# FedericoCos/PathTracer_GaussianSplatting

Hardware: AMD Instinct MI355X
Metric: Mrays/s (path trace) + Gsplats/s (3DGS) at 1920×1080, 1/2/4/8 MI355X (higher is better)
Workload: dtype f32; 1 GPU; C3 path trace: 250000-tri Sponza-like atrium, 1920x1080, 64 spp per GPU; width=1920, height=1080, spp_per_gpu=64, triangles=250000, bvh_nodes=58627, bvh_depth=13, bvh_build=host binned SAH, 103.2 ms, parallelism=single GPU

## Files before the change

### pathtracer_gaussiansplatting_amd/csrc/api.cpp

```cpp
#ifndef PTGS_BVH_LEAF
#define PTGS_BVH_LEAF 3
#endif
#include <hip/hip_runtime.h>

#include <algorithm>
#include <chrono>
#include <cmath>
#include <cstdarg>
#include <cstdio>
#include <cstring>
#include <string>
#include <vector>

#include "../../include/ptgs/ptgs.h"
#include "bvh.h"
#include "bvh_gpu.h"
#include "knn.h"
#include "hostmath.h"
#include "pt_launch.h"
#include "pt_wavefront.h"
#include "comm.h"
#include "splat.h"
#include "splat_backward.h"
#include "splat_sh.h"
// ... 396 lines not shown
      (void)hipFree(g.tri_flags);
    } else {
      (void)hipFree(g.nodes);
      (void)hipFree(g.tris);
      (void)hipFree(g.tri_flags);
      return fail(c, PTGS_EHIP, "GPU BVH build: %s", hipGetErrorString(e));
    }
  }
  if (!built) {
    auto t0 = std::chrono::steady_clock::now();
    BvhOut bvh;
    std::vector<float> n4;
    uint32_t num4 = 0, dep4 = 0, need = PTGS_STACK_TOTAL;
    int built_leaf = -1;
    bool fits = false;
    uint32_t built_depth = 0;
    for (const BvhTry& tr : bvh_tries()) {
      if (tr.leaf != built_leaf || tr.depth != built_depth) {
        build_bvh(tris, tr.leaf, tr.depth, bvh);
        built_leaf = tr.leaf;
        built_depth = tr.depth;
        if (bvh.depth >= PTGS_STACK) return fail(c, PTGS_ERANGE, "BVH depth %u exceeds the traversal stack", bvh.depth);
      }
      fits = collapse_fit(bvh.nodes, n4, num4, dep4, tr.fan, need);
      bvh_log("host", tr.leaf, tr.fan, tr.depth, dep4, need);
      if (fits) break;
    }
    auto t1 = std::chrono::steady_clock::now();
    if (!fits) return fail(c, PTGS_ERANGE, "BVH depth %u exceeds the traversal stack", bvh.depth);
    s.deep_stack = need >= PTGS_STACK ? 1 : 0;
    if ((rc = upload(c, (const float4*)n4.data(), n4.size() / 4, &s.nodes))) return rc;
    host_n4.swap(n4);
    bvh.num_nodes = num4;
    bvh.depth = dep4;
    if ((rc = upload(c, (const float4*)bvh.tris.data(), bvh.tris.size() / 4, &s.tris))) return rc;
    if ((rc = upload(c, bvh.tri_flags.data(), bvh.tri_flags.size(), &s.tri_flags))) return rc;
    c->info.num_bvh_nodes = bvh.num_nodes;
    c->info.bvh_depth = bvh.depth;
    c->info.max_leaf_size = bvh.max_leaf;
    c->info.build_ms = std::chrono::duration<double, std::milli>(t1 - t0).count();
  }
  if (c->info.num_bvh_nodes > bvh_node_limit())
    return fail(c, PTGS_ERANGE, "BVH of %u 4-wide nodes exceeds the traversal's 2 GiB node window (%u nodes)",
                c->info.num_bvh_nodes, bvh_node_limit());
  {
    const size_t nf = (size_t)c->info.num_bvh_nodes * 32;
    if (host_n4.size() != nf) {
      host_n4.resize(nf);
      HIPCHK(c, hipMemcpy(host_n4.data(), s.nodes, nf * sizeof(float), hipMemcpyDeviceToHost));
    }
    std::vector<uint32_t> n64;
    if (!quantize_bvh4(host_n4.data(), c->info.num_bvh_nodes, n64))
      return fail(c, PTGS_ERANGE, "BVH node extents beyond the compact nodes' step range (2^-100 .. 2^100)");
    if ((rc = upload(c, (const uint4*)n64.data(), n64.size() / 4, &s.nodes64))) return rc;
  }
  ptgs_vertex dummy_v{};
  uint32_t dummy_i = 0;
  ptgs_mesh_info dummy_m{};
  if ((rc = upload(c, d->num_vertices ? d->vertices : &dummy_v, d->num_vertices ? d->num_vertices : 1, &s.vertices))) return rc;
  if ((rc = upload(c, d->num_indices ? d->indices : &dummy_i, d->num_indices ? d->num_indices : 1, &s.indices))) return rc;
  if ((rc = upload(c, d->num_meshes ? d->meshes : &dummy_m, d->num_meshes ? d->num_meshes : 1, &s.meshes))) return rc;
  if ((rc = upload(c, d->materials, d->num_materials, &s.materials))) return rc;
  {
    const uint32_t zero4[4] = {0, 0, 0, 0};
    if ((rc = upload(c, (const uint4*)(hitrec.empty() ? zero4 : hitrec.data()), hitrec.empty() ? 1 : hitrec.size() / 4,
                     &s.hitrec)))
      return rc;
  }
  if ((rc = upload(c, d->light_triangles, d->num_light_triangles, &s.light_tris))) return rc;
  if ((rc = upload(c, d->light_cdf, d->num_light_cdf, &s.light_cdf))) return rc;
  if ((rc = upload(c, d->punctual_lights, d->num_punctual_lights, &s.plights))) return rc;
  if ((rc = upload(c, d->punctual_cdf, d->num_punctual_cdf, &s.pcdf))) return rc;
  if ((rc = upload(c, (const float4*)d->blue_noise_rgba32f, (size_t)bn * bn, &s.blue_noise))) return rc;
  if ((rc = upload(c, texpool.texels.data(), texpool.texels.size(), &s.tex.texels))) return rc;
  if ((rc = upload(c, texpool.info.data(), texpool.info.size(), &s.tex.info))) return rc;
  if ((rc = upload(c, texpool.lut.data(), texpool.lut.size(), &s.tex.lut))) return rc;
  s.tex.count = d->num_textures;
  s.uses_textures = 0;
  for (uint32_t i = 0; i < d->num_materials; ++i) {
    const ptgs_material& m = d->materials[i];
    if (m.albedo_texture_index > 0 || m.normal_texture_index > 0 || m.metallic_roughness_texture_index > 0 ||
        m.emissive_texture_index > 0 || m.clearcoat_texture_index > 0 || m.clearcoat_roughness_texture_index > 0 ||
        m.sg_id > 0)
      s.uses_textures = 1;
  }
  s.num_light_cdf = d->num_light_cdf;
  s.num_plights = d->num_punctual_lights;
  s.bn_size = (int32_t)bn;
  s.has_transparent = has_transparent ? 1 : 0;
  c->dsc = s;
  c->has_scene = true;
  c->info.num_triangles = (uint32_t)tris.size();
  return PTGS_OK;
}

int ptgs_scene_get_info(const ptgs_ctx* c, ptgs_scene_info* out) {
  if (!c || !out) return PTGS_EINVAL;
  if (!c->has_scene) return PTGS_ENOSCENE;
  *out = c->info;
  return PTGS_OK;
}

int ptgs_scene_get_bvh(const ptgs_ctx* c, ptgs_bvh_buffers* out) {
  if (!c || !out) return PTGS_EINVAL;
  if (!c->has_scene) return PTGS_ENOSCENE;
  out->nodes = (const float*)c->dsc.nodes;
// ... 585 lines not shown
```

### pathtracer_gaussiansplatting_amd/csrc/bvh.cpp

```cpp
#include "bvh.h"

#include <algorithm>
#include <cmath>
#include <cstring>
#include <limits>

#ifndef PTGS_BVH_CT
#define PTGS_BVH_CT 0.125f
#endif
#ifndef PTGS_BVH_BINS
#define PTGS_BVH_BINS 32
#endif

namespace ptgs {

namespace {

struct Box {
  float lo[3], hi[3];
  void reset() {
    for (int a = 0; a < 3; ++a) { lo[a] = std::numeric_limits<float>::infinity(); hi[a] = -lo[a]; }
  }
  void grow(const float* p) {
    for (int a = 0; a < 3; ++a) { lo[a] = std::min(lo[a], p[a]); hi[a] = std::max(hi[a], p[a]); }
// ... 289 lines not shown
    const float* f = &n4[32 * (size_t)i];
    uint32_t* o = &out[PTGS_NODE64_DWORDS * (size_t)i];
    bool real[4];
    for (int j = 0; j < 4; ++j) {
      real[j] = true;
      for (int a = 0; a < 3; ++a) {
        const float lo = f[(2 * a) * 4 + j], hi = f[(2 * a + 1) * 4 + j];
        if (!(std::fabs(lo) < kFar && std::fabs(hi) < kFar && lo <= hi)) real[j] = false;
      }
    }
    for (int a = 0; a < 3; ++a) {
      const float* lo = f + (2 * a) * 4;
      const float* hi = f + (2 * a + 1) * 4;
      float lmin = std::numeric_limits<float>::infinity(), hmax = -lmin;
      for (int j = 0; j < 4; ++j)
        if (real[j]) { lmin = std::min(lmin, lo[j]); hmax = std::max(hmax, hi[j]); }
      float org = 0.0f, step = 1.0f;
      uint32_t wlo = 0xffffffffu, whi = 0u;
      if (lmin <= hmax) {
        org = std::nextafterf((float)((double)lmin - m), -std::numeric_limits<float>::infinity());
        int e = (int)std::ceil(std::log2(std::max(((double)hmax + m - (double)org) / 255.0, 1e-300)));
        e = std::max(e, -100);
        for (;; ++e) {
          if (e > 100) return false;
          step = std::ldexp(1.0f, e);
          bool fits = true;
          wlo = 0xffffffffu; whi = 0u;
          for (int j = 0; j < 4 && fits; ++j) {
            if (!real[j]) continue;
            const double tl = (double)lo[j] - m, th = (double)hi[j] + m;
            double ql = std::floor((tl - (double)org) / (double)step);
            ql = std::min(std::max(ql, 0.0), 255.0);
            while (ql > 0.0 && (double)std::fmaf((float)ql, step, org) > tl) ql -= 1.0;
            double qh = std::ceil((th - (double)org) / (double)step);
            qh = std::min(std::max(qh, 0.0), 256.0);
            while (qh <= 255.0 && (double)std::fmaf((float)qh, step, org) < th) qh += 1.0;
            if (qh > 255.0) { fits = false; break; }
            wlo = (wlo & ~(0xffu << (8 * j))) | ((uint32_t)ql << (8 * j));
            whi |= (uint32_t)qh << (8 * j);
          }
          if (fits) break;
        }
      }
      std::memcpy(&o[a], &org, 4);
      std::memcpy(&o[3 + a], &step, 4);
      o[6 + 2 * a] = wlo;
      o[7 + 2 * a] = whi;
    }
    std::memcpy(&o[12], &f[24], 16);
  }
  return true;
}

}
```

### pathtracer_gaussiansplatting_amd/csrc/bvh.h

```cpp
#pragma once

#include <stdint.h>
#include <vector>

namespace ptgs {

struct BuildTri {
  float v0[3], v1[3], v2[3];
  uint32_t mesh, prim, gid;
  uint32_t flags;
};

struct BvhOut {
  std::vector<float> nodes;
  std::vector<float> tris;
  std::vector<uint32_t> tri_flags;
  uint32_t num_nodes = 0;
  uint32_t depth = 0;
  uint32_t max_leaf = 0;
};

void build_bvh(const std::vector<BuildTri>& tris, int max_leaf_size, uint32_t max_depth, BvhOut& out);

void collapse_bvh4(const std::vector<float>& nodes2, std::vector<float>& nodes4, uint32_t& num_nodes4,
                   uint32_t& max_stack, uint32_t& depth4, int max_children = 4);

#define PTGS_NODE64_DWORDS 16
bool quantize_bvh4(const float* nodes4, uint32_t num_nodes, std::vector<uint32_t>& out);

}
```

### pathtracer_gaussiansplatting_amd/csrc/pt_device.h

```cpp
#pragma once

#include <hip/hip_runtime.h>
#include "detmath.h"
#include "texture.h"
#include "../../include/ptgs/ptgs.h"

namespace ptgs {

struct DevScene {
  const float4* nodes;
  const uint4* nodes64;
  const float4* tris;
  const uint32_t* tri_flags;
  const ptgs_vertex* vertices;
  const uint32_t* indices;
  const ptgs_mesh_info* meshes;
  const ptgs_material* materials;
  const uint4* hitrec;
  const ptgs_light_triangle* light_tris;
  const ptgs_light_cdf* light_cdf;
  const ptgs_punctual_light* plights;
  const ptgs_punctual_cdf* pcdf;
  const float4* blue_noise;
  DevTextures tex;
  int32_t uses_textures;
  int32_t deep_stack;
  uint32_t num_light_cdf;
  uint32_t num_plights;
  int32_t bn_size;
  int32_t has_transparent;
};

struct CamParams {
  float inv_view[16];
  float inv_proj[16];
  float ambient[4];
  float emissive_flux, punctual_flux, p_emissive;
  float fov, win_height, use_lod, lod_factor;
};

struct Hit {
  float t, u, v;
  uint32_t gid;
  uint32_t slot;
};

struct TraversalCounters {
  uint32_t nodes;
  uint32_t tris;
  uint32_t hits;
#ifdef PT_LANES
  struct PtLaneCounts* lanes_p;
#endif
};

enum PtLoop { PT_L_NODE = 0, PT_L_LEAF, PT_L_TRI, PT_L_ANY_NODE, PT_L_ANY_TRI, PT_L_BOUNCE, PT_L_SAMPLE, PT_L_COUNT };
#ifdef PT_LANES
__device__ unsigned long long g_pt_lanes[2 * PT_L_COUNT];
struct PtLaneCounts {
  uint32_t w[PT_L_COUNT], l[PT_L_COUNT];
};
__device__ __forceinline__ void pt_lane_tick(PtLaneCounts& c, int i) {
  const unsigned long long ex = __builtin_amdgcn_read_exec();
  c.l[i] += 1u;
  if (__lane_id() == (uint32_t)__builtin_ctzll(ex)) c.w[i] += 1u;
}
__device__ __forceinline__ void pt_lanes_flush(const PtLaneCounts& c) {
  for (int i = 0; i < PT_L_COUNT; ++i) {
    atomicAdd(&g_pt_lanes[2 * i], (unsigned long long)c.w[i]);
    atomicAdd(&g_pt_lanes[2 * i + 1], (unsigned long long)c.l[i]);
  }
}
#define PT_LANE_TICK(cnt, i) pt_lane_tick(*(cnt).lanes_p, (i))
#define PT_LANES_INIT(tc) PtLaneCounts tc##_lanes = {}; (tc).lanes_p = &tc##_lanes
#define PT_LANES_FLUSH(tc) pt_lanes_flush(tc##_lanes)
#else
#define PT_LANE_TICK(cnt, i) ((void)0)
#define PT_LANES_INIT(tc) ((void)0)
#define PT_LANES_FLUSH(tc) ((void)0)
#endif

#ifndef PTGS_STACK
#define PTGS_STACK 39
// ... 51 lines not shown
#if PTGS_PT_NEARFAR
  r.nx = r.inv.x < 0.0f ? 16u : 0u;
  r.ny = r.inv.y < 0.0f ? 48u : 32u;
  r.nz = r.inv.z < 0.0f ? 80u : 64u;
#endif
  return r;
}

__device__ __forceinline__ bool tri_isect(const Ray& r, v3 v0, v3 e1, v3 e2, float& t, float& u, float& v) {
  v3 pvec = cross3(r.d, e2);
  float det = dot3(e1, pvec);
  if (det == 0.0f) return false;
  float inv_det = 1.0f / det;
  v3 tvec = r.o - v0;
  u = dot3(tvec, pvec) * inv_det;
  if (u < 0.0f || u > 1.0f) return false;
  v3 qvec = cross3(tvec, e1);
  v = dot3(r.d, qvec) * inv_det;
  if (v < 0.0f || u + v > 1.0f) return false;
  t = dot3(e2, qvec) * inv_det;
  return true;
}

template <bool TEX>
__device__ __forceinline__ bool anyhit_accept(const DevScene& sc, uint32_t mesh, uint32_t prim, float u, float v,
                                              uint32_t seed, uint32_t gid) {
  const ptgs_mesh_info info = sc.meshes[mesh];
  const ptgs_material& m = sc.materials[info.material_index];
  float alpha_cutoff = m.alpha_cutoff;
  bool is_blend = m.pad > 0.5f;
  if (alpha_cutoff == 0.0f && !is_blend) return true;
  float alpha = m.base_color_factor[3];
  if (TEX && m.albedo_texture_index > 0) {
    const uint32_t i0 = sc.indices[info.index_offset + prim * 3u + 0u];
    const uint32_t i1 = sc.indices[info.index_offset + prim * 3u + 1u];
    const uint32_t i2 = sc.indices[info.index_offset + prim * 3u + 2u];
    const ptgs_vertex& v0 = sc.vertices[info.vertex_offset + i0];
    const ptgs_vertex& v1 = sc.vertices[info.vertex_offset + i1];
    const ptgs_vertex& v2 = sc.vertices[info.vertex_offset + i2];
    const float bx = (1.0f - u) - v;
    const float tu = (v0.tex_coord[0] * bx + v1.tex_coord[0] * u) + v2.tex_coord[0] * v;
    const float tv = (v0.tex_coord[1] * bx + v1.tex_coord[1] * u) + v2.tex_coord[1] * v;
    alpha = alpha * sample_texture(sc.tex, m.albedo_texture_index, tu, tv, 0.0f).w;
  }
  if (alpha_cutoff > 0.0f) return !(alpha < alpha_cutoff);
  return !(alpha_hash(seed, gid) > alpha);
}

__device__ __noinline__ bool anyhit_accept_call(const DevScene& sc, uint32_t mesh, uint32_t prim, float u, float v,
                                                uint32_t seed, uint32_t gid) {
  return anyhit_accept<true>(sc, mesh, prim, u, v, seed, gid);
}

template <bool STATS, bool TEX, bool AH_CALL = false>
__device__ __forceinline__ void leaf_closest(const DevScene& sc, const Ray& r, int leaf, Hit& h,
                                             uint32_t seed, TraversalCounters& cnt) {
  uint32_t L = (uint32_t)(~leaf);
  uint32_t start = L & 0x07ffffffu;
  uint32_t count = (L >> 27) + 1u;
  float4 na = sc.tris[3u * start], nb = sc.tris[3u * start + 1u], nc = sc.tris[3u * start + 2u];
  for (uint32_t k = 0; k < count; ++k) {
    PT_LANE_TICK(cnt, PT_L_TRI);
    float4 a = na, b = nb, c = nc;
    asm volatile("" : "+v"(a.x), "+v"(a.y), "+v"(a.z), "+v"(a.w), "+v"(b.x), "+v"(b.y), "+v"(b.z), "+v"(b.w),
                      "+v"(c.x), "+v"(c.y), "+v"(c.z), "+v"(c.w));
    if (k + 1 < count) {
      const float4* tn = sc.tris + 3u * (start + k + 1u);
      na = tn[0]; nb = tn[1]; nc = tn[2];
    }
    if (STATS) cnt.tris++;
    float t, u, v;
    if (!tri_isect(r, mk3(a.x, a.y, a.z), mk3(b.x, b.y, b.z), mk3(c.x, c.y, c.z), t, u, v)) continue;
    if (!(t >= r.tmin && t <= h.t)) continue;
    uint32_t gid = f2u(c.w);
    if (t == h.t && gid >= h.gid) continue;
    if (sc.has_transparent && (sc.tri_flags[start + k] & 1u)) {
      const bool acc = (AH_CALL && TEX) ? anyhit_accept_call(sc, f2u(a.w), f2u(b.w), u, v, seed, gid)
                                        : anyhit_accept<TEX>(sc, f2u(a.w), f2u(b.w), u, v, seed, gid);
      if (!acc) continue;
    }
    h.t = t; h.u = u; h.v = v; h.gid = gid; h.slot = start + k;
  }
}

struct Box4 {
  float tn[4];
  int c[4];
  unsigned long long hm[4];
};
#if PTGS_PT_NEARFAR
__device__ __forceinline__ float4 node_ld(__amdgpu_buffer_rsrc_t rs, uint32_t off) {
  typedef unsigned int u4 __attribute__((ext_vector_type(4)));
  const u4 v = __builtin_amdgcn_raw_buffer_load_b128(rs, (int)off, 0, 0);
  return make_float4(__uint_as_float(v.x), __uint_as_float(v.y), __uint_as_float(v.z), __uint_as_float(v.w));
}
__device__ __forceinline__ void box4(const Ray& r, const DevScene& sc, int node, float tcap, Box4& o) {
  const __amdgpu_buffer_rsrc_t rs = __builtin_amdgcn_make_buffer_rsrc((void*)sc.nodes, 0, 0x7fffffff, 0x00020000);
  const uint32_t base = (uint32_t)node << 7;
  const uint32_t ox = base + r.nx, oy = base + r.ny, oz = base + r.nz;
  const float4 nx = node_ld(rs, ox), fx = node_ld(rs, ox ^ 16u);
  const float4 ny = node_ld(rs, oy), fy = node_ld(rs, oy ^ 16u);
  const float4 nz = node_ld(rs, oz), fz = node_ld(rs, oz ^ 16u);
  float4 ch = node_ld(rs, base + 96u);
  asm volatile("" : "+v"(ch.x), "+v"(ch.y), "+v"(ch.z), "+v"(ch.w));
  const float NX[4] = {nx.x, nx.y, nx.z, nx.w}, FX[4] = {fx.x, fx.y, fx.z, fx.w};
  const float NY[4] = {ny.x, ny.y, ny.z, ny.w}, FY[4] = {fy.x, fy.y, fy.z, fy.w};
  const float NZ[4] = {nz.x, nz.y, nz.z, nz.w}, FZ[4] = {fz.x, fz.y, fz.z, fz.w};
  const float CH[4] = {ch.x, ch.y, ch.z, ch.w};
#pragma unroll
  for (int j = 0; j < 4; ++j) {
    const float x0 = __builtin_fmaf(NX[j], r.inv.x, -r.oinv.x), x1 = __builtin_fmaf(FX[j], r.inv.x, -r.oinv.x);
    const float y0 = __builtin_fmaf(NY[j], r.inv.y, -r.oinv.y), y1 = __builtin_fmaf(FY[j], r.inv.y, -r.oinv.y);
// ... 59 lines not shown
  u4 ch = __builtin_amdgcn_raw_buffer_load_b128(rs, (int)(base + 48u), 0, 0);
  asm volatile("" : "+v"(ch.x), "+v"(ch.y), "+v"(ch.z), "+v"(ch.w));
  const float sx = __uint_as_float(a.w) * r.inv.x, sy = __uint_as_float(b.x) * r.inv.y, sz = __uint_as_float(b.y) * r.inv.z;
  const float cx = __builtin_fmaf(__uint_as_float(a.x), r.inv.x, -r.oinv.x);
  const float cy = __builtin_fmaf(__uint_as_float(a.y), r.inv.y, -r.oinv.y);
  const float cz = __builtin_fmaf(__uint_as_float(a.z), r.inv.z, -r.oinv.z);
#if PTGS_PT_NEARFAR
  const bool gx = (r.nx & 16u) != 0u, gy = (r.ny & 16u) != 0u, gz = (r.nz & 16u) != 0u;
#else
  const bool gx = r.inv.x < 0.0f, gy = r.inv.y < 0.0f, gz = r.inv.z < 0.0f;
#endif
  const uint32_t nX = gx ? b.w : b.z, fX = gx ? b.z : b.w;
  const uint32_t nY = gy ? p.y : p.x, fY = gy ? p.x : p.y;
  const uint32_t nZ = gz ? p.w : p.z, fZ = gz ? p.z : p.w;
  const uint32_t CH[4] = {ch.x, ch.y, ch.z, ch.w};
#pragma unroll
  for (int j = 0; j < 4; ++j) {
    const float x0 = __builtin_fmaf(node64_q(nX, j), sx, cx), x1 = __builtin_fmaf(node64_q(fX, j), sx, cx);
    const float y0 = __builtin_fmaf(node64_q(nY, j), sy, cy), y1 = __builtin_fmaf(node64_q(fY, j), sy, cy);
    const float z0 = __builtin_fmaf(node64_q(nZ, j), sz, cz), z1 = __builtin_fmaf(node64_q(fZ, j), sz, cz);
    const float tn = fmaxf(fmaxf(x0, y0), fmaxf(z0, r.tmin));
#if PTGS_PT_ASM_MIN
    float tf;
    asm("v_min3_f32 %0, %1, %2, %3" : "=v"(tf) : "v"(x1), "v"(y1), "v"(z1));
    asm("v_min_f32 %0, %1, %2" : "=v"(tf) : "v"(tf), "v"(tcap));
#else
    const float tf = fminf(fminf(x1, y1), fminf(z1, tcap));
#endif
    unsigned long long hm = __builtin_amdgcn_ballot_w64(tn <= tf * 1.0000004f);
    if (j >= 2) hm &= __builtin_amdgcn_ballot_w64(CH[j] != 0u);
    o.tn[j] = __builtin_amdgcn_inverse_ballot_w64(hm) ? tn : __builtin_huge_valf();
    o.c[j] = (int)CH[j];
    o.hm[j] = hm;
  }
}
template <bool N64>
__device__ __forceinline__ void box4_sel(const Ray& r, const DevScene& sc, int node, float tcap, Box4& o) {
  if (N64) box4_q(r, sc, node, tcap, o);
  else box4(r, sc, node, tcap, o);
}
__device__ __forceinline__ void cswap4(Box4& b, int i, int j) {
  const bool sw = b.tn[j] < b.tn[i];
  const float ti = b.tn[i], tj = b.tn[j];
  const int ci = b.c[i], cj = b.c[j];
  b.tn[i] = sw ? tj : ti; b.tn[j] = sw ? ti : tj;
  b.c[i] = sw ? cj : ci; b.c[j] = sw ? ci : cj;
}
template <typename Push, typename Pop>
__device__ __forceinline__ int enter_box4(Box4& b, Push push, Pop pop) {
  const unsigned long long h0 = b.hm[0], h1 = b.hm[1], h2 = b.hm[2], h3 = b.hm[3];
  if (!__builtin_amdgcn_inverse_ballot_w64(h0 | h1 | h2 | h3)) return pop();
  cswap4(b, 0, 1); cswap4(b, 2, 3); cswap4(b, 0, 2); cswap4(b, 1, 3); cswap4(b, 1, 2);
  const unsigned long long a01 = h0 & h1, o01 = h0 | h1, a23 = h2 & h3, o23 = h2 | h3;
  if (__builtin_amdgcn_inverse_ballot_w64(a01 & a23)) push(b.c[3]);
  if (__builtin_amdgcn_inverse_ballot_w64((a01 & o23) | (o01 & a23))) push(b.c[2]);
  if (__builtin_amdgcn_inverse_ballot_w64(a01 | a23 | (o01 & o23))) push(b.c[1]);
  return b.c[0];
}

template <bool STATS, bool TEX, int SS = PTGS_BLOCK, int OVF = PTGS_STACK_OVF, bool N64 = false>
__device__ __forceinline__ Hit trace_closest(const DevScene& sc, const Ray& r, uint32_t seed, int* stack,
                                             TraversalCounters& cnt) {
  Hit h; h.t = r.tmax; h.u = 0.f; h.v = 0.f; h.gid = 0xffffffffu; h.slot = 0;
  const Ray rq = node64_ray<N64>(r);
  int sp = 0;
  int node = 0;
  const int DONE = 0x7fffffff;
  int leaf = DONE;
  int ovf[OVF > 0 ? OVF : 1];
  auto push = [&](int x) {
    if (OVF == 0 || sp < PTGS_STACK) stack[sp * SS] = x;
    else ovf[sp - PTGS_STACK] = x;
    ++sp;
  };
  auto pop = [&]() -> int {
    if (!sp) return DONE;
    --sp;
    return (OVF == 0 || sp < PTGS_STACK) ? stack[sp * SS] : ovf[sp - PTGS_STACK];
  };
  for (;;) {
    while (node >= 0 && node != DONE) {
      PT_LANE_TICK(cnt, PT_L_NODE);
      Box4 b;
      box4_sel<N64>(rq, sc, node, h.t, b);
      if (STATS) cnt.nodes += 4;
      node = enter_box4(b, push, pop);
      if (node < 0 && leaf == DONE) {
        leaf = node;
        node = pop();
      }
      if ((__builtin_amdgcn_ballot_w64(leaf != DONE) | __builtin_amdgcn_ballot_w64(node == DONE)) ==
          __builtin_amdgcn_read_exec())
        break;
    }
    if (leaf != DONE) {
      PT_LANE_TICK(cnt, PT_L_LEAF);
      leaf_closest<STATS, TEX>(sc, r, leaf, h, seed, cnt);
      leaf = DONE;
    }
    if (node < 0) {
      leaf_closest<STATS, TEX>(sc, r, node, h, seed, cnt);
      node = pop();
    }
    if (node == DONE) return h;
  }
}

template <bool STATS, bool TEX, int SS = PTGS_BLOCK, int OVF = PTGS_STACK_OVF, bool N64 = false>
__device__ __forceinline__ bool trace_any(const DevScene& sc, const Ray& r, uint32_t seed, int* stack,
                                          TraversalCounters& cnt) {
  const Ray rq = node64_ray<N64>(r);
  int sp = 0;
  int node = 0;
  int ovf[OVF > 0 ? OVF : 1];
  auto pop_nz = [&]() -> int {
    --sp;
    return (OVF == 0 || sp < PTGS_STACK) ? stack[sp * SS] : ovf[sp - PTGS_STACK];
  };
  while (true) {
    while (node >= 0) {
      PT_LANE_TICK(cnt, PT_L_ANY_NODE);
      Box4 b;
      box4_sel<N64>(rq, sc, node, r.tmax, b);
      if (STATS) cnt.nodes += 4;
      int next = -0x7fffffff - 1;
      bool have = false;
#pragma unroll
      for (int j = 0; j < 4; ++j)
        if (b.tn[j] != __builtin_huge_valf()) {
          if (!have) {
            next = b.c[j];
            have = true;
          } else {
            if (OVF == 0 || sp < PTGS_STACK) stack[sp * SS] = b.c[j];
            else ovf[sp - PTGS_STACK] = b.c[j];
            ++sp;
          }
        }
      if (!have) {
        if (sp == 0) return false;
        node = pop_nz();
        continue;
      }
      node = next;
    }
    uint32_t L = (uint32_t)(~node);
    uint32_t start = L & 0x07ffffffu;
    uint32_t count = (L >> 27) + 1u;
    for (uint32_t k = 0; k < count; ++k) {
      PT_LANE_TICK(cnt, PT_L_ANY_TRI);
      const float4* tp = sc.tris + 3u * (start + k);
      float4 a = tp[0], bb = tp[1], c = tp[2];
      if (STATS) cnt.tris++;
      float t, u, v;
      if (!tri_isect(r, mk3(a.x, a.y, a.z), mk3(bb.x, bb.y, bb.z), mk3(c.x, c.y, c.z), t, u, v)) continue;
      if (!(t >= r.tmin && t <= r.tmax)) continue;
      if (sc.has_transparent && (sc.tri_flags[start + k] & 1u)) {
        if (!anyhit_accept<TEX>(sc, f2u(a.w), f2u(bb.w), u, v, seed, f2u(c.w))) continue;
      }
      return true;
    }
    if (sp == 0) return false;
    node = pop_nz();
  }
}

__device__ __forceinline__ v4 matvec(const float* m, v4 v) {
  return mk4(((m[0] * v.x + m[4] * v.y) + m[8] * v.z) + m[12] * v.w,
             ((m[1] * v.x + m[5] * v.y) + m[9] * v.z) + m[13] * v.w,
             ((m[2] * v.x + m[6] * v.y) + m[10] * v.z) + m[14] * v.w,
             ((m[3] * v.x + m[7] * v.y) + m[11] * v.z) + m[15] * v.w);
}

__device__ __forceinline__ float4 blue_noise_texel(const DevScene& sc, uint32_t lx, uint32_t ly, uint32_t frame) {
  const float a1 = 0.75487766624669276f;
  const float a2 = 0.56984029099805327f;
  float rx = fractx((float)frame * a1);
  float ry = fractx((float)frame * a2);
  int ox = (int)(rx * (float)sc.bn_size);
  int oy = (int)(ry * (float)sc.bn_size);
  int px = ((int)lx + ox) & (sc.bn_size - 1);
  int py = ((int)ly + oy) & (sc.bn_size - 1);
  return sc.blue_noise[py * sc.bn_size + px];
}

__device__ __forceinline__ void primary_ray(const DevScene& sc, const CamParams& cp, uint32_t x, uint32_t y,
                                            uint32_t W, uint32_t H, uint32_t frame, v3& ro, v3& rd, float4& blue,
                                            uint32_t& seed) {
  blue = blue_noise_texel(sc, x, y, frame);
  seed = (y * W + x) + frame * 719393u;
  const float pcx = (float)x + blue.x, pcy = (float)y + blue.y;
  const float ux = pcx / (float)W, uy = pcy / (float)H;
  const float dx = ux * 2.0f - 1.0f, dy = uy * 2.0f - 1.0f;
  const v4 origin = matvec(cp.inv_view, mk4(0.f, 0.f, 0.f, 1.f));
  const v4 target = matvec(cp.inv_proj, mk4(dx, dy, 1.f, 1.f));
  const v3 dirc = normalize3(mk3(target.x, target.y, target.z) / target.w);
  const v4 direction = matvec(cp.inv_view, mk4(dirc.x, dirc.y, dirc.z, 0.f));
  ro = mk3(origin.x, origin.y, origin.z);
  rd = normalize3(mk3(direction.x, direction.y, direction.z));
}

// ... 270 lines not shown
```

### pathtracer_gaussiansplatting_amd/csrc/pt_kernels.hip

```cpp
#include <hip/hip_runtime.h>

#include "pt_shade.h"
#include "pt_launch.h"
#include "xcd.h"

#ifndef PTGS_PT_XCD_REMAP
#define PTGS_PT_XCD_REMAP 0
#endif
#ifndef PTGS_PT_WG
#define PTGS_PT_WG 64
#endif
#ifndef PTGS_PT_PAIR
#define PTGS_PT_PAIR 1
#endif
#ifndef PTGS_PT_LPP
#define PTGS_PT_LPP 2
#endif
#ifndef PTGS_PT_SCHED
#define PTGS_PT_SCHED 1
#endif
#ifndef PTGS_PT_SCHED_MIN
#define PTGS_PT_SCHED_MIN (1u << 22)
#endif

// ... 76 lines not shown
  const bool active = (x < W) && (y < row1);

  __shared__ int s_stack[PTGS_STACK * PTGS_PT_WG];
  ShadeCtx c; c.sc = &sc; c.cp = &cp; c.stack = s_stack + threadIdx.x; c.shadow_rays = 0;
  TraversalCounters tc; tc.nodes = 0; tc.tris = 0; tc.hits = 0;
  PT_LANES_INIT(tc);
  uint32_t ext_rays = 0, samples = 0;

  const size_t pix = (size_t)y * W + x;
  v3 state = mk3(0.0f);
  float state_a = 0.0f;
  if (active && half == 0u && (mode == PTGS_ACCUM_SUM || frame0 > 0)) {
    float4 prev = accum[pix];
    state = mk3(prev.x, prev.y, prev.z);
    state_a = prev.w;
  }
  auto fold = [&](const v3& acc, uint32_t s) {
    const uint32_t frame = frame0 + s * stride;
    if (mode == PTGS_ACCUM_SUM) {
      state = state + acc;
      state_a = state_a + 1.0f;
    } else if (frame > 0) {
      float blend = 1.0f / (float)(frame + 1u);
      state = mix3(state, acc, blend);
    } else {
      state = acc;
    }
  };
  const uint32_t iters = (spp + lpp - 1u) / lpp;
  for (uint32_t k = 0; k < iters; ++k) {
    const uint32_t s = k * lpp + half;
    v3 acc = mk3(0.0f);
    if (active && s < spp) {
      PT_LANE_TICK(tc, PT_L_SAMPLE);
      const uint32_t frame = frame0 + s * stride;
      v3 ro, rd;
      float4 blue;
      uint32_t seed;
      primary_ray(sc, cp, x, y, W, H, frame, ro, rd, blue, seed);

      v3 thr = mk3(1.0f);
      Payload p;
      p.seed = seed;
      p.blue = mk2(blue.z, blue.w);
      p.last_pdf = 0.0f;
      p.hit_flag = 0.0f;
      p.color = mk3(0.0f); p.weight = mk3(1.0f); p.next_o = ro; p.next_d = rd;
      int max_depth = 12;
      for (int depth = 0; depth < max_depth; ++depth) {
        PT_LANE_TICK(tc, PT_L_BOUNCE);
        p.depth = depth;
        Ray ray = make_ray(ro, rd, 0.001f, 10000.0f);
        ext_rays++;
        Hit h = trace_closest<STATS, TEX, PTGS_PT_WG, DEEP ? PTGS_STACK_OVF : 0, PTGS_PT_NODE64 != 0>(sc, ray, p.seed, c.stack, tc);
        if (STATS && h.gid != 0xffffffffu) tc.hits++;
        ShadowQuery q;
        q.flags = 0;
        if (h.gid == 0xffffffffu) miss<false>(cp, p);
        else closest_hit<false, TEX>(c, p, ray, h, q);
        resolve_shadow<STATS, TEX, PTGS_PT_WG, DEEP ? PTGS_STACK_OVF : 0, PTGS_PT_NODE64 != 0>(c, p.color, p.seed, q, tc);
        acc = acc + p.color * thr;
        acc = vmin(acc, 5.0f);
        if (p.hit_flag < 0.0f) break;
        if (depth == 0 && p.hit_flag < 1.5f) max_depth = 4;
        thr = thr * p.weight;
        ro = p.next_o;
        rd = p.next_d;
        float mt = fmaxx(fmaxx(thr.x, thr.y), thr.z);
        if (mt < 0.001f) break;
        if (depth >= 4) {
          float pr = clampf(mt, 0.05f, 0.95f);
          if (rnd(p.seed) > pr) break;
          thr = thr / pr;
        }
      }
      samples++;
    }
    if (pair) {
      v3 got[4];
      got[0] = acc;
#pragma unroll
      for (uint32_t j = 1; j < 4; ++j) {
        const int src = (int)((lane + j * pw) & 63u);
        got[j] = mk3(__shfl(acc.x, src), __shfl(acc.y, src), __shfl(acc.z, src));
        if (j + 1u >= lpp) break;
      }
      if (active && half == 0u) {
#pragma unroll
        for (uint32_t j = 0; j < 4; ++j)
          if (j < lpp && s + j < spp) fold(got[j], s + j);
      }
    } else if (active) {
      fold(acc, s);
    }
  }
  if (active && half == 0u) {
    if (mode == PTGS_ACCUM_SUM) accum[pix] = make_float4(state.x, state.y, state.z, state_a);
    else accum[pix] = make_float4(state.x, state.y, state.z, 1.0f);
  }
  flush_counters(counters, ext_rays, c.shadow_rays, samples, tc, STATS);
  PT_LANES_FLUSH(tc);
#if !PTGS_PT_XCD_REMAP
  if (cost) {
    __syncthreads();
    if (lid == 0) cost[by * gridDim.x + bx] = (uint32_t)min(__builtin_amdgcn_s_memrealtime() - t_start, 0xFFFFFFFFull);
  }
#endif
// ... 273 lines not shown
```

### pathtracer_gaussiansplatting_amd/csrc/pt_wavefront.hip

```cpp
#include <hip/hip_runtime.h>

#include <algorithm>
#include <cstdlib>

#include "pt_shade.h"
#include "pt_wavefront.h"

namespace ptgs {

namespace {

constexpr int WF_DONE = 0x7fffffff;
constexpr uint32_t WF_MAX_DEPTH = 12;
constexpr uint8_t WF_EXT = 1u, WF_SHADOW = 2u;
constexpr uint32_t WF_RING = 128u;
constexpr uint32_t WF_NCNT = 6;

__device__ __forceinline__ uint32_t lane_id() { return threadIdx.x & 63u; }

__device__ __forceinline__ uint32_t mbcnt64(unsigned long long m) {
  return __builtin_amdgcn_mbcnt_hi((uint32_t)(m >> 32), __builtin_amdgcn_mbcnt_lo((uint32_t)m, 0u));
}

__device__ __forceinline__ void wave_sync() {
// ... 91 lines not shown
    uint32_t t = 0;
    for (uint32_t w = 0; w < blockDim.x / 64u; ++w) t += s_red[w];
    part[k * stride + blockIdx.x] += t;
  }
}

}

__global__ __launch_bounds__(256) void pt_wf_raygen_kernel(DevScene sc, CamParams cp, WfArgs a) {
  __shared__ uint32_t s_red[4];
  const uint32_t slot = blockIdx.x * 256u + threadIdx.x;
  uint32_t x, y, frame;
  slot_pixel(a, slot, x, y, frame);
  const bool valid = slot < a.slots && x < a.W && y < a.row1;
  if (valid) {
    v3 ro, rd;
    float4 blue;
    uint32_t seed;
    primary_ray(sc, cp, x, y, a.W, a.H, frame, ro, rd, blue, seed);
    stnt(a.ray_o + slot, make_float4(ro.x, ro.y, ro.z, u2f(seed)));
    stnt(a.ray_d + slot, make_float4(rd.x, rd.y, rd.z, 0.0f));
    stnt(a.st_thr + slot, make_float4(1.0f, 1.0f, 1.0f, 0.0f));
    stnt(a.st_w + slot, make_float4(1.0f, 1.0f, 1.0f, 0.0f));
    stnt(a.st_acc + slot, make_float4(0.0f, 0.0f, 0.0f, (float)WF_MAX_DEPTH));
  }
  if (slot < a.slots) a.flags[slot] = valid ? WF_EXT : 0u;
  if (blockIdx.x == 0 && threadIdx.x < 2u * (WF_MAX_DEPTH + 1u)) a.live[threadIdx.x] = threadIdx.x == 0 ? 1u : 0u;
  block_count(a.part, a.part_stride, 2, valid ? 1u : 0u, s_red);
}

template <bool STATS, bool TEX>
__global__ __launch_bounds__(256, wf_min_waves(PTGS_WF_LDS_EXT)) void pt_wf_extend_kernel(DevScene sc, WfArgs a, uint32_t depth, uint32_t per_wave,
                                                              uint32_t refill) {
  if (a.live[2u * depth] == 0u) return;
  __shared__ int s_stack[PTGS_WF_LDS_EXT * PTGS_BLOCK];
  __shared__ uint16_t s_ring[4][WF_RING];
  uint32_t* s_red = reinterpret_cast<uint32_t*>(s_ring);
  TravStack<PTGS_WF_LDS_EXT> st;
  st.lds = s_stack + threadIdx.x;
  st.ovf = a.ovf + blockIdx.x * 256u + threadIdx.x;
  st.ostride = gridDim.x * 256u;
  st.sp = 0;
  const uint32_t begin = (blockIdx.x * 4u + (threadIdx.x >> 6)) * per_wave;
  SlotStream ss;
  ss_init(ss, s_ring[threadIdx.x >> 6], begin, min(a.slots, begin + per_wave));
  TraversalCounters tc; tc.nodes = 0; tc.tris = 0; tc.hits = 0;
  PT_LANES_INIT(tc);
  uint32_t traced = 0;
  bool active = false;
  uint32_t slot = 0, seed = 0;
  Ray r = make_ray(mk3(0.0f), mk3(1.0f), 0.001f, 10000.0f);
  Hit h; h.t = 0.f; h.u = 0.f; h.v = 0.f; h.gid = 0xffffffffu; h.slot = 0;
  int node = WF_DONE, leaf = WF_DONE;
  auto push = [&](int v) { st.push(v); };
  auto pop = [&]() -> int { return st.sp ? st.pop_nz() : WF_DONE; };
  for (;;) {
    const unsigned long long idle = __ballot(!active);
    const uint32_t nidle = (uint32_t)__popcll(idle);
    if (nidle >= refill || nidle == 64u || idle == __ballot(true)) {
      ss_fill(ss, a.flags, WF_EXT, nidle);
      const uint32_t avail = ss.tail - ss.head, rk = mbcnt64(idle);
      if (!active && rk < avail) {
        slot = ss.at(ss.head + rk);
        const float4 ro = ldnt(a.ray_o + slot), rd = ldnt(a.ray_d + slot);
        r = make_ray(mk3(ro.x, ro.y, ro.z), mk3(rd.x, rd.y, rd.z), 0.001f, 10000.0f);
        seed = f2u(ro.w);
        h.t = r.tmax; h.u = 0.f; h.v = 0.f; h.gid = 0xffffffffu;
        node = 0; st.sp = 0; leaf = WF_DONE;
        active = true;
      }
      ss.head += min(avail, nidle);
      if (!active) break;
    }
    if (!active) continue;
    while (node >= 0 && node != WF_DONE) {
      Box4 b;
      box4(r, sc, node, h.t, b);
      if (STATS) tc.nodes += 4;
      node = enter_box4(b, push, pop);
      if (node < 0 && leaf == WF_DONE) {
        leaf = node;
        node = pop();
      }
      if ((__builtin_amdgcn_ballot_w64(leaf != WF_DONE) | __builtin_amdgcn_ballot_w64(node == WF_DONE)) ==
          __builtin_amdgcn_read_exec())
        break;
    }
    if (leaf != WF_DONE) {
      leaf_closest<STATS, TEX, PTGS_WF_AH_CALL_EXT>(sc, r, leaf, h, seed, tc);
      leaf = WF_DONE;
    }
    if (node < 0) {
      leaf_closest<STATS, TEX, PTGS_WF_AH_CALL_EXT>(sc, r, node, h, seed, tc);
      node = pop();
    }
    if (node == WF_DONE) {
      stnt(a.hits + slot, make_float4(h.t, h.u, h.v, u2f(h.gid)));
      if (STATS && h.gid != 0xffffffffu) tc.hits++;
      traced++;
      active = false;
    }
  }
  block_count(a.part, a.part_stride, 0, traced, s_red);
  if (STATS) {
    block_count(a.part, a.part_stride, 3, tc.nodes, s_red);
    block_count(a.part, a.part_stride, 4, tc.tris, s_red);
    block_count(a.part, a.part_stride, 5, tc.hits, s_red);
// ... 353 lines not shown
```

Baseline: 5802 Mrays/s.

## Pack child entry distance into traversal stack words to cull stale pops

Repacks the compact BVH node links so that leaf start and count use only as many bits as the scene needs. The spare high bits of each stack word then hold the truncated entry distance of the pushed child. On pop, entries whose stored bound lies beyond the current closest hit are discarded without fetching the node, which removes wasted node loads and box tests after the hit distance shrinks. In exchange, every push and pop does extra mask work and pop runs a loop. The leaf decode now depends on runtime layout fields, and the key width depends on how many link bits the scene leaves free.

```diff
diff --git a/pathtracer_gaussiansplatting_amd/csrc/api.cpp b/pathtracer_gaussiansplatting_amd/csrc/api.cpp
--- a/pathtracer_gaussiansplatting_amd/csrc/api.cpp
+++ b/pathtracer_gaussiansplatting_amd/csrc/api.cpp
@@ -472,6 +472,16 @@
     std::vector<uint32_t> n64;
     if (!quantize_bvh4(host_n4.data(), c->info.num_bvh_nodes, n64))
       return fail(c, PTGS_ERANGE, "BVH node extents beyond the compact nodes' step range (2^-100 .. 2^100)");
+    int force = -1;
+    if (const char* e = getenv("PTGS_PT_STACK_KEY_BITS")) force = std::max(0, atoi(e));
+    const StackLayout sl = stack_layout(host_n4.data(), c->info.num_bvh_nodes, force);
+    pack_links64(n64, c->info.num_bvh_nodes, sl);
+    s.stk_key_mask = sl.key_mask;
+    s.leaf_shift = sl.leaf_shift;
+    s.leaf_start_mask = sl.leaf_start_mask;
+    if (getenv("PTGS_BVH_LOG"))
+      fprintf(stderr, "[ptgs] stack word:%u link bits, %u key bits (mask %08x), leaf shift %u\n", sl.ref_bits, sl.key_bits,
+              sl.key_mask, sl.leaf_shift);
     if ((rc = upload(c, (const uint4*)n64.data(), n64.size() / 4, &s.nodes64))) return rc;
   }
   ptgs_vertex dummy_v{};
diff --git a/pathtracer_gaussiansplatting_amd/csrc/bvh.cpp b/pathtracer_gaussiansplatting_amd/csrc/bvh.cpp
--- a/pathtracer_gaussiansplatting_amd/csrc/bvh.cpp
+++ b/pathtracer_gaussiansplatting_amd/csrc/bvh.cpp
@@ -365,4 +365,40 @@
   return true;
 }
 
-}
+static uint32_t bits_for(uint32_t v) {
+  uint32_t b = 0;
+  while (v) { ++b; v >>= 1; }
+  return b;
+}
+
+StackLayout stack_layout(const float* n4, uint32_t num, int force_key_bits) {
+  uint32_t max_start = 0, max_cm1 = 0;
+  for (uint32_t i = 0; i < num; ++i)
+    for (int j = 0; j < 4; ++j) {
+      int32_t link;
+      std::memcpy(&link, &n4[32 * (size_t)i + 24 + j], 4);
+      if (link >= 0) continue;
+      const uint32_t L = ~(uint32_t)link;
+      max_start = std::max(max_start, L & 0x07ffffffu);
+      max_cm1 = std::max(max_cm1, L >> 27);
+    }
+  StackLayout l;
+  l.leaf_shift = bits_for(max_start);
+  l.leaf_start_mask = (1u << l.leaf_shift) - 1u;
+  const uint32_t payload = std::max(bits_for(num), l.leaf_shift + bits_for(max_cm1));
+  l.ref_bits = payload + 1u;
+  const uint32_t room = 32u - l.ref_bits;
+  l.key_bits = force_key_bits >= 0 ? std::min((uint32_t)force_key_bits, room) : (room >= PTGS_STACK_KEY_MIN ? room : 0u);
+  l.key_mask = stack_key_mask(l.key_bits);
+  return l;
+}
+
+void pack_links64(std::vector<uint32_t>& n64, uint32_t num, const StackLayout& l) {
+  for (uint32_t i = 0; i < num; ++i)
+    for (int j = 0; j < 4; ++j) {
+      uint32_t& w = n64[PTGS_NODE64_DWORDS * (size_t)i + 12 + j];
+      w = stack_link_pack((int32_t)w, l);
+    }
+}
+
+}
diff --git a/pathtracer_gaussiansplatting_amd/csrc/bvh.h b/pathtracer_gaussiansplatting_amd/csrc/bvh.h
--- a/pathtracer_gaussiansplatting_amd/csrc/bvh.h
+++ b/pathtracer_gaussiansplatting_amd/csrc/bvh.h
@@ -2,6 +2,8 @@
 
 #include <stdint.h>
 #include <vector>
+
+#include "stack_key.h"
 
 namespace ptgs {
 
@@ -28,4 +30,8 @@
 #define PTGS_NODE64_DWORDS 16
 bool quantize_bvh4(const float* nodes4, uint32_t num_nodes, std::vector<uint32_t>& out);
 
+#define PTGS_STACK_KEY_MIN 8
+StackLayout stack_layout(const float* nodes4, uint32_t num_nodes, int force_key_bits = -1);
+void pack_links64(std::vector<uint32_t>& nodes64, uint32_t num_nodes, const StackLayout& layout);
+
 }
diff --git a/pathtracer_gaussiansplatting_amd/csrc/pt_device.h b/pathtracer_gaussiansplatting_amd/csrc/pt_device.h
--- a/pathtracer_gaussiansplatting_amd/csrc/pt_device.h
+++ b/pathtracer_gaussiansplatting_amd/csrc/pt_device.h
@@ -3,6 +3,7 @@
 #include <hip/hip_runtime.h>
 #include "detmath.h"
 #include "texture.h"
+#include "stack_key.h"
 #include "../../include/ptgs/ptgs.h"
 
 namespace ptgs {
@@ -29,6 +30,9 @@
   uint32_t num_plights;
   int32_t bn_size;
   int32_t has_transparent;
+  uint32_t stk_key_mask;
+  uint32_t leaf_shift;
+  uint32_t leaf_start_mask;
 };
 
 struct CamParams {
@@ -186,12 +190,23 @@
   return anyhit_accept<true>(sc, mesh, prim, u, v, seed, gid);
 }
 
-template <bool STATS, bool TEX, bool AH_CALL = false>
+template <bool PK>
+__device__ __forceinline__ void leaf_range(const DevScene& sc, int leaf, uint32_t& start, uint32_t& count) {
+  if (PK) {
+    start = (uint32_t)leaf & sc.leaf_start_mask;
+    count = (((uint32_t)leaf & 0x7fffffffu) >> sc.leaf_shift) + 1u;
+  } else {
+    const uint32_t L = (uint32_t)(~leaf);
+    start = L & 0x07ffffffu;
+    count = (L >> 27) + 1u;
+  }
+}
+
+template <bool STATS, bool TEX, bool AH_CALL = false, bool PK = false>
 __device__ __forceinline__ void leaf_closest(const DevScene& sc, const Ray& r, int leaf, Hit& h,
                                              uint32_t seed, TraversalCounters& cnt) {
-  uint32_t L = (uint32_t)(~leaf);
-  uint32_t start = L & 0x07ffffffu;
-  uint32_t count = (L >> 27) + 1u;
+  uint32_t start, count;
+  leaf_range<PK>(sc, leaf, start, count);
   float4 na = sc.tris[3u * start], nb = sc.tris[3u * start + 1u], nc = sc.tris[3u * start + 2u];
   for (uint32_t k = 0; k < count; ++k) {
     PT_LANE_TICK(cnt, PT_L_TRI);
@@ -357,31 +372,49 @@
   if (!__builtin_amdgcn_inverse_ballot_w64(h0 | h1 | h2 | h3)) return pop();
   cswap4(b, 0, 1); cswap4(b, 2, 3); cswap4(b, 0, 2); cswap4(b, 1, 3); cswap4(b, 1, 2);
   const unsigned long long a01 = h0 & h1, o01 = h0 | h1, a23 = h2 & h3, o23 = h2 | h3;
-  if (__builtin_amdgcn_inverse_ballot_w64(a01 & a23)) push(b.c[3]);
-  if (__builtin_amdgcn_inverse_ballot_w64((a01 & o23) | (o01 & a23))) push(b.c[2]);
-  if (__builtin_amdgcn_inverse_ballot_w64(a01 | a23 | (o01 & o23))) push(b.c[1]);
+  if (__builtin_amdgcn_inverse_ballot_w64(a01 & a23)) push(b.c[3], b.tn[3]);
+  if (__builtin_amdgcn_inverse_ballot_w64((a01 & o23) | (o01 & a23))) push(b.c[2], b.tn[2]);
+  if (__builtin_amdgcn_inverse_ballot_w64(a01 | a23 | (o01 & o23))) push(b.c[1], b.tn[1]);
   return b.c[0];
 }
 
-template <bool STATS, bool TEX, int SS = PTGS_BLOCK, int OVF = PTGS_STACK_OVF, bool N64 = false>
+#ifndef PTGS_PT_STACK_CULL
+#define PTGS_PT_STACK_CULL 1
+#endif
+template <bool STATS, bool TEX, int SS = PTGS_BLOCK, int OVF = PTGS_STACK_OVF, bool N64 = false, bool CULL = false>
 __device__ __forceinline__ Hit trace_closest(const DevScene& sc, const Ray& r, uint32_t seed, int* stack,
                                              TraversalCounters& cnt) {
+  static_assert(!CULL || N64, "the distance key needs the compact nodes' packed links");
   Hit h; h.t = r.tmax; h.u = 0.f; h.v = 0.f; h.gid = 0xffffffffu; h.slot = 0;
   const Ray rq = node64_ray<N64>(r);
   int sp = 0;
   int node = 0;
-  const int DONE = 0x7fffffff;
+  const uint32_t kmask = sc.stk_key_mask;
+  const int DONE = CULL ? (int)(0x7fffffffu & ~kmask) : 0x7fffffff;
   int leaf = DONE;
   int ovf[OVF > 0 ? OVF : 1];
-  auto push = [&](int x) {
+  auto push = [&](int c, float tn) {
+    const int x = CULL ? (int)stack_pack((uint32_t)c, tn, kmask) : c;
     if (OVF == 0 || sp < PTGS_STACK) stack[sp * SS] = x;
     else ovf[sp - PTGS_STACK] = x;
     ++sp;
   };
   auto pop = [&]() -> int {
-    if (!sp) return DONE;
-    --sp;
-    return (OVF == 0 || sp < PTGS_STACK) ? stack[sp * SS] : ovf[sp - PTGS_STACK];
+    if (!CULL) {
+      if (!sp) return DONE;
+      --sp;
+      return (OVF == 0 || sp < PTGS_STACK) ? stack[sp * SS] : ovf[sp - PTGS_STACK];
+    }
+    const float cap = h.t * 1.0000004f;
+    uint32_t x;
+    do {
+      x = (uint32_t)DONE;
+      if (sp) {
+        --sp;
+        x = (uint32_t)((OVF == 0 || sp < PTGS_STACK) ? stack[sp * SS] : ovf[sp - PTGS_STACK]);
+      }
+    } while (stack_bound(x, kmask) > cap);
+    return (int)stack_link(x, kmask);
   };
   for (;;) {
     while (node >= 0 && node != DONE) {
@@ -400,11 +433,11 @@
     }
     if (leaf != DONE) {
       PT_LANE_TICK(cnt, PT_L_LEAF);
-      leaf_closest<STATS, TEX>(sc, r, leaf, h, seed, cnt);
+      leaf_closest<STATS, TEX, false, N64>(sc, r, leaf, h, seed, cnt);
       leaf = DONE;
     }
     if (node < 0) {
-      leaf_closest<STATS, TEX>(sc, r, node, h, seed, cnt);
+      leaf_closest<STATS, TEX, false, N64>(sc, r, node, h, seed, cnt);
       node = pop();
     }
     if (node == DONE) return h;
@@ -449,9 +482,8 @@
       }
       node = next;
     }
-    uint32_t L = (uint32_t)(~node);
-    uint32_t start = L & 0x07ffffffu;
-    uint32_t count = (L >> 27) + 1u;
+    uint32_t start, count;
+    leaf_range<N64>(sc, node, start, count);
     for (uint32_t k = 0; k < count; ++k) {
       PT_LANE_TICK(cnt, PT_L_ANY_TRI);
       const float4* tp = sc.tris + 3u * (start + k);
diff --git a/pathtracer_gaussiansplatting_amd/csrc/pt_kernels.hip b/pathtracer_gaussiansplatting_amd/csrc/pt_kernels.hip
--- a/pathtracer_gaussiansplatting_amd/csrc/pt_kernels.hip
+++ b/pathtracer_gaussiansplatting_amd/csrc/pt_kernels.hip
@@ -152,7 +152,8 @@
         p.depth = depth;
         Ray ray = make_ray(ro, rd, 0.001f, 10000.0f);
         ext_rays++;
-        Hit h = trace_closest<STATS, TEX, PTGS_PT_WG, DEEP ? PTGS_STACK_OVF : 0, PTGS_PT_NODE64 != 0>(sc, ray, p.seed, c.stack, tc);
+        Hit h = trace_closest<STATS, TEX, PTGS_PT_WG, DEEP ? PTGS_STACK_OVF : 0, PTGS_PT_NODE64 != 0,
+                              PTGS_PT_NODE64 != 0 && PTGS_PT_STACK_CULL != 0>(sc, ray, p.seed, c.stack, tc);
         if (STATS && h.gid != 0xffffffffu) tc.hits++;
         ShadowQuery q;
         q.flags = 0;
diff --git a/pathtracer_gaussiansplatting_amd/csrc/pt_wavefront.hip b/pathtracer_gaussiansplatting_amd/csrc/pt_wavefront.hip
--- a/pathtracer_gaussiansplatting_amd/csrc/pt_wavefront.hip
+++ b/pathtracer_gaussiansplatting_amd/csrc/pt_wavefront.hip
@@ -167,7 +167,7 @@
   Ray r = make_ray(mk3(0.0f), mk3(1.0f), 0.001f, 10000.0f);
   Hit h; h.t = 0.f; h.u = 0.f; h.v = 0.f; h.gid = 0xffffffffu; h.slot = 0;
   int node = WF_DONE, leaf = WF_DONE;
-  auto push = [&](int v) { st.push(v); };
+  auto push = [&](int v, float) { st.push(v); };
   auto pop = [&]() -> int { return st.sp ? st.pop_nz() : WF_DONE; };
   for (;;) {
     const unsigned long long idle = __ballot(!active);
diff --git a/pathtracer_gaussiansplatting_amd/csrc/stack_key.h b/pathtracer_gaussiansplatting_amd/csrc/stack_key.h
--- /dev/null
+++ b/pathtracer_gaussiansplatting_amd/csrc/stack_key.h
@@ -0,0 +1,49 @@
+#pragma once
+
+#include <stdint.h>
+
+#if defined(__HIPCC__) || defined(__CUDACC__)
+#define PTGS_SK_HD __host__ __device__ inline __attribute__((always_inline))
+#else
+#define PTGS_SK_HD inline
+#endif
+
+namespace ptgs {
+
+struct StackLayout {
+  uint32_t key_mask;
+  uint32_t leaf_shift;
+  uint32_t leaf_start_mask;
+  uint32_t key_bits;
+  uint32_t ref_bits;
+};
+
+PTGS_SK_HD uint32_t stack_key_mask(uint32_t w) { return w >= 31u ? 0x7fffffffu : (((1u << w) - 1u) << (31u - w)); }
+
+PTGS_SK_HD uint32_t stack_f2u(float f) {
+  uint32_t u;
+  __builtin_memcpy(&u, &f, 4);
+  return u;
+}
+PTGS_SK_HD float stack_u2f(uint32_t u) {
+  float f;
+  __builtin_memcpy(&f, &u, 4);
+  return f;
+}
+
+PTGS_SK_HD uint32_t stack_pack(uint32_t link, float tn, uint32_t key_mask) { return (stack_f2u(tn) & key_mask) | link; }
+PTGS_SK_HD float stack_bound(uint32_t word, uint32_t key_mask) { return stack_u2f(word & key_mask); }
+PTGS_SK_HD uint32_t stack_link(uint32_t word, uint32_t key_mask) { return word & ~key_mask; }
+
+PTGS_SK_HD uint32_t stack_link_pack(int32_t link, const StackLayout& l) {
+  if (link >= 0) return (uint32_t)link;
+  const uint32_t L = ~(uint32_t)link;
+  return 0x80000000u | (L & 0x07ffffffu) | ((L >> 27) << l.leaf_shift);
+}
+PTGS_SK_HD int32_t stack_link_unpack(uint32_t p, const StackLayout& l) {
+  if (!(p & 0x80000000u)) return (int32_t)p;
+  const uint32_t u = p & 0x7fffffffu;
+  return (int32_t)~((u & l.leaf_start_mask) | ((u >> l.leaf_shift) << 27));
+}
+
+}
```

New measurement: 6087 Mrays/s, median of 6. 1.05x the previous value.
